# duanyiqun/DiffusionDepth

Hardware: AMD Instinct MI355X
Metric: depth-maps/sec (20-step DDIM, KITTI 352x1216 f16r, B=4 maps per GPU per step; depth RMSE vs the reference's CPU path <= 1e-3 on this workload AND at KITTI's depth range 0-80 m: see cpu_baseline.rmse_gate) (higher is better)
Workload: dtype f16 (f16 MFMA operands, fp32 accumulation; refined mode: f16-pair weights in conv1 / conv4 / conv3(cond), block-scaled int16 hand-over of y3 and conv3(cond)); 1 GPU; kitti 352x1216 image -> latent 16x176x608, cond 256x176x608, Res head denoiser (mmbev_res50 config), T=20, encoder+loop+decoder, inputs resident in HBM; global_batch=4, parallelism=dp1 (independent images, no collective), ranks_seen=1, streams=2, graph=True, variant=res

## Files before the change

### diffusiondepth_amd/csrc/dd_api.cpp

```cpp
#include "dd_api_internal.h"
#include <cstdlib>

namespace ddapi {
thread_local std::string g_create_error;
}


extern "C" {

const char* dd_version(void) { return "ddepth 0.1 gfx950 (hip, mfma bf16/f16/f32 implicit-GEMM conv3x3+GN+ReLU, hipGraph DDIM loop)"; }

const char* dd_last_error(dd_handle_t h) { return h ? h->err.c_str() : g_create_error.c_str(); }

int dd_create(dd_handle_t* out, int device, int variant) {
  if (!out) { g_create_error = "dd_create: out is NULL"; return DD_ERR_INVALID_ARG; }
  *out = nullptr;
  if (variant != DD_VARIANT_RES && variant != DD_VARIANT_SWIN) { g_create_error = "dd_create: unknown variant"; return DD_ERR_INVALID_ARG; }
  int n = 0;
  hipError_t e = hipGetDeviceCount(&n);
  if (e != hipSuccess || n <= 0) {
    g_create_error = std::string("dd_create: no HIP device available (") + (e != hipSuccess ? hipGetErrorString(e) : "count = 0") +
                     "); this library has no CPU fallback";
    return DD_ERR_HIP;
  }
// ... 90 lines not shown
      DD_HIP(hipDeviceSynchronize());
      h->plans.clear(); h->last_once_plan = nullptr;
      h->cond_bufs.clear(); h->fpn_cond.reset(); h->fpn_cond_key[3] = -1; h->fpn_out.reset(); h->fpn_work.reset();
    }
    h->bf16_pure = value != 0;
  }
  else if (k == "naive_wgrad") h->naive_wgrad = value != 0;
  else if (k == "lane_probe") h->lane_probe = value != 0;
  else if (k == "x3_grad_fp32") h->x3_grad_fp32 = value != 0;
  else if (k == "keep_trajectory") h->keep_traj = value != 0;
  else if (k == "use_trajectory") h->use_traj = value;
  else if (k == "adjoint_tiled") h->adjoint_tiled = value != 0;
  else if (k == "streams") h->n_streams = value < 1 ? 1 : (int)value;
  else if (k == "keep_activations_mb") h->keep_act_mb = value < 0 ? 0 : value;
  else if (k == "big_tiles") {
    if (value < -1 || value > 1) return h->fail(DD_ERR_INVALID_ARG, "dd_set_option: big_tiles must be -1 (automatic), 0 or 1");
    if (h->big_tiles != (int)value) { DD_HIP(hipDeviceSynchronize()); h->plans.clear(); h->last_once_plan = nullptr; }
    h->big_tiles = (int)value;
  }
  else if (k == "thin_slots") {
    if (value < 1 || value > 4096) return h->fail(DD_ERR_INVALID_ARG, "dd_set_option: thin_slots must be in [1, 4096]");
    if (h->thin_slots != (int)value) { DD_HIP(hipDeviceSynchronize()); h->plans.clear(); h->last_once_plan = nullptr; }
    h->thin_slots = (int)value;
  }
  else if (k == "one_buffer") {
    if (value < 0 || value > 2) return h->fail(DD_ERR_INVALID_ARG, "dd_set_option: one_buffer must be 0, 1 or 2");
    if (h->one_buffer != (int)value) { DD_HIP(hipDeviceSynchronize()); h->plans.clear(); h->last_once_plan = nullptr; }
    h->one_buffer = (int)value;
  }
  else if (k == "cond_direct") {
    if (value < 0 || value > 1) return h->fail(DD_ERR_INVALID_ARG, "dd_set_option: cond_direct must be 0 or 1");
    h->cond_direct = (int)value;
  }
  else if (k == "cond_split") {
    if (value < 0 || value > 1) return h->fail(DD_ERR_INVALID_ARG, "dd_set_option: cond_split must be 0 or 1");
    h->cond_split = (int)value;
  }
  else if (k == "thin_stream") {
    if (value < 0 || value > 1) return h->fail(DD_ERR_INVALID_ARG, "dd_set_option: thin_stream must be 0 or 1");
    if (h->thin_stream != (int)value) {
      DD_HIP(hipDeviceSynchronize());
      h->plans.clear(); h->last_once_plan = nullptr;
    }
    h->thin_stream = (int)value;
  }
  else if (k == "f16r_wide" || k == "f16r_p4" || k == "f16r_c1") {
    if (value < 0 || value > 1) return h->fail(DD_ERR_INVALID_ARG, "dd_set_option: " + k + " must be 0 or 1");
    int& opt = k == "f16r_wide" ? h->f16r_wide : k == "f16r_c1" ? h->f16r_c1 : h->f16r_p4;
    if (opt != (int)value) { DD_HIP(hipDeviceSynchronize()); h->plans.clear(); h->last_once_plan = nullptr; }
    opt = (int)value;
  }
  else if (k == "phase_prof_buffer") h->prof_buf = reinterpret_cast<unsigned long long*>((uintptr_t)value);
  else if (k == "phase_prof_layer") h->prof_layer = (int)value;
  else if (k == "layer_timing") {
    drain_layer_events(h);
    h->layer_timing = value != 0;
    for (int i = 0; i < dd_handle_s::N_LAYER_SLOTS; ++i) { h->layer_ms[i] = 0; h->layer_cnt[i] = 0; }
  } else return h->fail(DD_ERR_INVALID_ARG, "dd_set_option: unknown key '" + k + "'");
  return DD_OK;
}

int dd_get_counter(dd_handle_t h, const char* key, int64_t* value) {
  if (!h || !key || !value) return DD_ERR_INVALID_ARG;
  const std::string k(key);
  if (k == "graph_launches") *value = h->n_graph_launches;
  else if (k == "graph_default") *value = h->graph_off_by_env ? 0 : 1;
  else if (k == "eager_loops") *value = h->n_eager_loops;
  else if (k == "graph_capture_failures") *value = h->n_capture_failures;
  else if (k == "plans") *value = (int64_t)h->plans.size();
  else if (k == "neck_launches") *value = h->n_neck_launches;
  else if (k == "trajectory_ticket") *value = h->traj_serial;
  else if (k == "lane_calls") *value = h->n_lane_calls;
  else if (k == "lane_probe_retries") *value = h->n_lane_probe_retries;
  else if (k == "lane_overlap") *value = h->lane_overlap_seen;
  else if (k == "cond_split_ok") *value = (h->fpn_committed && h->fpn_split_ok ? 1 : 0) | (h->neck_committed && h->neck_split_ok ? 2 : 0);
  else if (k == "resident_slots") *value = h->resident_slots;
  else if (k == "trajectory_reuses") *value = h->n_traj_reuse;
  else if (k == "thin_stream_launches") *value = h->thin_stream_launches;
  else if (k.compare(0, 13, "kid_launches:") == 0) {
    int id = 0;
    const size_t n = k.size() - 13;
    bool ok = n >= 1 && n <= 3 && !(n > 1 && k[13] == '0');
    for (size_t i = 13; ok && i < k.size(); ++i) { ok = k[i] >= '0' && k[i] <= '9'; id = id * 10 + (k[i] - '0'); }
    if (!ok || !kid_listed(id)) return h->fail(DD_ERR_INVALID_ARG, "dd_get_counter: '" + k + "' does not name a kernel id (dd_kernel_ids.h)");
    *value = h->kid_launches[id];
  }
  else return h->fail(DD_ERR_INVALID_ARG, "dd_get_counter: unknown key '" + k + "'");
  return DD_OK;
}

int dd_get_layer_ms(dd_handle_t h, int layer, double* total_ms, int64_t* launches) {
  if (!h || layer < 1 || layer > dd_handle_s::N_LAYER_SLOTS || !total_ms || !launches) return DD_ERR_INVALID_ARG;
  drain_layer_events(h);
  *total_ms = h->layer_ms[layer - 1];
  *launches = h->layer_cnt[layer - 1];
  return DD_OK;
}

int dd_last_loop_ms(dd_handle_t h, float* ms) {
  if (!h || !ms) return DD_ERR_INVALID_ARG;
  *ms = 0.f;
  if (!h->ev_valid) return DD_OK;
  DD_HIP(hipEventSynchronize(h->ev1));
  DD_HIP(hipEventElapsedTime(ms, h->ev0, h->ev1));
  return DD_OK;
// ... 425 lines not shown
  }
  h->last_once_plan = pl;
  pl->traj_ticket = (h->keep_traj && precision != DD_PREC_NAIVE_FP32) ? ++h->traj_serial : 0;
  pl->traj_weights = h->weights_serial;
  if (h->debug_sync) DD_HIP(hipStreamSynchronize(s));
  return DD_OK;
}

int dd_add_noise(dd_handle_t h, const float* x0, const float* noise, const int64_t* t, float* out, int B, int C,
                 int lat_h, int lat_w, void* stream) {
  if (!h) return DD_ERR_INVALID_ARG;
  if (h->n_train <= 0) return h->fail(DD_ERR_STATE, "schedule not set (dd_set_schedule)");
  if (!x0 || !noise || !t || !out || B <= 0 || C <= 0 || lat_h <= 0 || lat_w <= 0)
    return h->fail(DD_ERR_INVALID_ARG, "dd_add_noise: null pointer or non-positive size");
  DD_HIP(hipSetDevice(h->device));
  DD_HIP(launch_add_noise(x0, noise, reinterpret_cast<const long long*>(t), h->d_acp.as<float>(), h->n_train, out, B,
                          (long long)C * lat_h * lat_w, reinterpret_cast<hipStream_t>(stream)));
  return DD_OK;
}

static int ensure_codec_tmp(dd_handle_t h, size_t bytes) {
  if (h->codec_tmp.bytes >= bytes) return DD_OK;
  DD_HIP(hipDeviceSynchronize());
  DD_HIP(h->codec_tmp.alloc(bytes));
  return DD_OK;
}

int dd_encode(dd_handle_t h, const float* depth, float* latent, int B, int H, int W, void* stream) {
  if (!h) return DD_ERR_INVALID_ARG;
  if (!h->codec_committed) return h->fail(DD_ERR_STATE, "depth_transform.* weights not committed");
  if (!depth || !latent || B <= 0 || H <= 0 || W <= 0) return h->fail(DD_ERR_INVALID_ARG, "dd_encode: null pointer or non-positive size");
  DD_HIP(hipSetDevice(h->device));
  const int lh = (H - 1) / 2 + 1, lw = (W - 1) / 2 + 1;
  int rc = ensure_codec_tmp(h, (size_t)B * lh * lw * LATENT_C * 4);
  if (rc) return rc;
  DD_HIP(launch_encode(h->codec, depth, h->codec_tmp.as<float>(), latent, B, H, W, reinterpret_cast<hipStream_t>(stream)));
  return DD_OK;
}

int dd_decode(dd_handle_t h, const float* latent, float* depth, int B, int lat_h, int lat_w, void* stream) {
  if (!h) return DD_ERR_INVALID_ARG;
  if (!h->codec_committed) return h->fail(DD_ERR_STATE, "depth_transform.* weights not committed");
  if (!latent || !depth || B <= 0 || lat_h <= 0 || lat_w <= 0) return h->fail(DD_ERR_INVALID_ARG, "dd_decode: null pointer or non-positive size");
  DD_HIP(hipSetDevice(h->device));
  int rc = ensure_codec_tmp(h, (size_t)B * (2 * lat_h) * (2 * lat_w) * LATENT_C * 4);
  if (rc) return rc;
  DD_HIP(launch_decode(h->codec, latent, h->codec_tmp.as<float>(), depth, B, lat_h, lat_w, reinterpret_cast<hipStream_t>(stream)));
  return DD_OK;
}

int dd_debug_fetch(dd_handle_t h, const char* name, float* out, int64_t numel, void* stream) {
  if (!h || !name || !out) return DD_ERR_INVALID_ARG;
  Plan* pl = h->last_once_plan;
  if (!pl) return h->fail(DD_ERR_STATE, "dd_debug_fetch: no dd_denoise_once call to inspect");
  const std::string n(name);
  const void* src = nullptr; int C = 0; int ek = store_kind(pl->ek);
  if (n == "y1") { src = pl->y1.p; C = HID_C; }
  else if (n == "y2") { src = pl->y2.p; C = COND_C; }
  else if (n == "y3") {
    src = pl->y3.p; C = HID_C;
    if (pl->ek == EK_F16R && pl->wide) return h->fail(DD_ERR_UNSUPPORTED, "dd_debug_fetch: y3 travels as scaled int16 in this plan (option f16r_wide = 1)");
  }
  else if (n == "y4") { src = pl->y4.p; C = LATENT_C; ek = EK_F32; }
  else return h->fail(DD_ERR_INVALID_ARG, "dd_debug_fetch: unknown tensor '" + n + "'");
  if (numel != (int64_t)pl->key.B * C * pl->key.h * pl->key.w) return h->fail(DD_ERR_INVALID_ARG, "dd_debug_fetch: numel mismatch");
  DD_HIP(launch_nhwc_to_nchw_f32(src, ek, out, pl->key.B, C, pl->key.h, pl->key.w, pl->key.prec != DD_PREC_NAIVE_FP32,
// ... 42 lines not shown
```

### diffusiondepth_amd/csrc/dd_api_internal.h

```cpp
#pragma once
#include "../../include/ddepth.h"
#include "dd_kernels.h"
#include "dd_kernel_ids.h"

#include <cmath>
#include <cstdio>
#include <cstring>
#include <map>
#include <memory>
#include <set>
#include <string>
#include <tuple>
#include <vector>

using namespace dd;

namespace ddapi {

extern thread_local std::string g_create_error;

struct DevBuf {
  void* p = nullptr;
  size_t bytes = 0;
  DevBuf() = default;
// ... 72 lines not shown
  int lane = 0;
  int lanes = 1;
  bool operator<(const PlanKey& o) const {
    return std::tie(B, h, w, ch, cw, T, prec, hoist, keep, lane, lanes) < std::tie(o.B, o.h, o.w, o.ch, o.cw, o.T, o.prec, o.hoist, o.keep, o.lane, o.lanes);
  }
};

struct Plan {
  PlanKey key{};
  int ek = EK_F32;
  DevBuf x[2];
  std::shared_ptr<DevBuf> cond;
  const void* cond_alias = nullptr;
  const void* graph_cond = nullptr;
  void* cond_ptr() const { return cond_alias ? const_cast<void*>(cond_alias) : (cond ? cond->p : nullptr); }
  DevBuf y1, y2, y3, y4;
  DevBuf a1, f, a3, eps;
  DevBuf sa, sf;
  DevBuf bX, bA1, bF, bA3;
  DevBuf bSa, bSf;
  DevBuf xstash;
  int64_t traj_ticket = 0;
  int64_t traj_weights = -1;
  bool traj_consumed = false;
  DevBuf gA, gY;
  DevBuf dgb;
  DevBuf bcorr;
  DevBuf ttab, tt_scratch;
  int64_t ttab_weights = -1;
  DevBuf ccond;
  DevBuf ccond_raw;
  DevBuf ccond_scale;
  DevBuf y3_scale;
  bool wide = false, c1 = false, p4 = false;
  DevBuf stats;
  DevBuf c1c2;
  DevBuf tsteps;
  std::vector<long long> tsteps_host;
  size_t stats_bytes = 0;
  hipGraphExec_t exec = nullptr;
  bool capture_failed = false;
  uint64_t last_use = 0;
  ~Plan() { if (exec) (void)hipGraphExecDestroy(exec); }
  int slots = 1;
  size_t kept_bytes = 0;
  void* slot(const DevBuf& b, int step) const { return static_cast<char*>(b.p) + (slots > 1 ? (size_t)step * (b.bytes / slots) : 0); }
  double* stat_ptr(int step, int layer) const {
    return stats.as<double>() + ((size_t)(step * 4 + layer) * key.B) * STAT_SLOTS * STAT_STRIDE;
  }
};

struct FpnWork {
  int B = 0, ek = -1, pyr = 0, hs[FPN_LEVELS] = {0}, ws[FPN_LEVELS] = {0};
  DevBuf fin[FPN_LEVELS];
  DevBuf lat[FPN_LEVELS];
  DevBuf up[FPN_LEVELS - 1];
  DevBuf pooled[FPN_LEVELS - 1];
  bool neck = false;
  DevBuf nk_cat[FPN_LEVELS];
  DevBuf nk_out[FPN_LEVELS];
};


struct NeckConv { int layer; std::string name; int cout, cin, ks, level, kind, C, Ck; };
constexpr int NECK_C_MPVIT[4] = {128, 216, 288, 288};
inline int neck_c(int pyr, int level) { return pyr == PYR_MPVIT ? NECK_C_MPVIT[level] : (192 << level); }
// ... 28 lines not shown
  ConvLayer L[4];
  ConvLayer LA, LB;
  DevBuf emb;
  DevBuf etab;
  DevBuf w5_oihw, w5pack[NUM_WIMG], pairp, kside;
  int64_t w5_weights = -1;
  int swin_w5 = 1;
  DevBuf zero_bias;
  int hoist_cond = -1;
  bool bf16_pure = false;
  DevBuf codec_buf;
  CodecWeights codec{};
  DevBuf codec_tmp;
  std::vector<float> acp;
  DevBuf d_acp;
  int n_train = 0;
  bool use_graph = true, timing = false, debug_sync = false, layer_timing = false;
  bool graph_off_by_env = false;
  int graph_fence = 0;
  bool train_graphs = false;
  int check_finite = 0;
  DevBuf chk_buf; std::vector<std::string> chk_labels;
  int ablate = 0;
  unsigned long long* prof_buf = nullptr;
  int prof_layer = 0;
  bool keep_traj = false;
  int64_t keep_act_mb = 65536;
  int n_streams = 1;
  int thin_slots = 512;
  int big_tiles = -1;
  int one_buffer = 1;
  int thin_stream = 1;
  int f16r_wide = 1;
  int f16r_c1 = 1;
  int f16r_p4 = 0;
  bool split_ok = true;
  DevBuf wmax;
  int resident_slots = 512;
  hipStream_t lane_stream[MAX_LANES] = {nullptr, nullptr, nullptr, nullptr};
  std::vector<hipEvent_t> probe_events;
  std::vector<hipStream_t> burnt_streams;
  int lane_probe = 1;
  int64_t n_lane_probe_retries = 0, lane_overlap_seen = -1;
  hipEvent_t lane_fork = nullptr, lane_done[MAX_LANES] = {nullptr, nullptr, nullptr, nullptr};
  int64_t n_lane_calls = 0;
  int active_lanes = 1;
  bool adjoint_tiled = true;
  int64_t traj_serial = 0, use_traj = 0, weights_serial = 0, n_traj_reuse = 0;
  int naive_wgrad = 0;
  int x3_grad_fp32 = 0;
  std::map<PlanKey, std::unique_ptr<Plan>> plans;
  DevBuf wgrad_ws[MAX_LANES];
  std::map<std::string, std::unique_ptr<DevBuf>> grads[MAX_LANES];
  std::map<std::tuple<int, int, int, int, int>, std::pair<std::shared_ptr<DevBuf>, uint64_t>> cond_bufs;
  bool neck_committed = false;
  DevBuf neck_w[NECK_CONVS][NUM_WIMG], neck_b[NECK_CONVS];
  int64_t n_neck_launches = 0;
  bool fpn_committed = false;
  int fpn_pyramid = PYR_DEFAULT;
  DevBuf fpn_lat_w[FPN_LEVELS][NUM_WIMG], fpn_lat_b[FPN_LEVELS];
  DevBuf fpn_up_w[FPN_LEVELS - 1][NUM_WIMG], fpn_up_b[FPN_LEVELS - 1];
  std::unique_ptr<FpnWork> fpn_work;
  std::shared_ptr<DevBuf> fpn_out;
  bool fpn_split_ok = false, neck_split_ok = false;
  int cond_direct = 1;
  int cond_split = 1;
  std::shared_ptr<DevBuf> fpn_cond;
  int fpn_cond_key[4] = {0, 0, 0, -1};
  uint64_t tick = 0;
  Plan* last_once_plan = nullptr;
  hipEvent_t ev0 = nullptr, ev1 = nullptr;
  bool ev_valid = false;
  hipStream_t cap_stream = nullptr;
  int64_t n_graph_launches = 0, n_eager_loops = 0, n_capture_failures = 0;
  static constexpr int N_LAYER_SLOTS = KID_LAST;
  double layer_ms[N_LAYER_SLOTS] = {0};
  int64_t layer_cnt[N_LAYER_SLOTS] = {0};
  std::vector<std::tuple<int, hipEvent_t, hipEvent_t>> pending_ev;
// ... 74 lines not shown
```

### diffusiondepth_amd/csrc/dd_api_plans.cpp

```cpp
#include "dd_api_internal.h"

namespace ddapi {

int check_common(dd_handle_t h, int B, int lh, int lw, int ch, int cw, bool need_schedule) {
  if (!h) return DD_ERR_INVALID_ARG;
  if (!h->committed) return h->fail(DD_ERR_STATE, "model.* weights not committed (call dd_set_weight for every key, then dd_commit_weights)");
  if (need_schedule && h->n_train <= 0) return h->fail(DD_ERR_STATE, "schedule not set (dd_set_schedule)");
  if (B <= 0 || lh <= 0 || lw <= 0) return h->fail(DD_ERR_INVALID_ARG, "B, lat_h, lat_w must be positive");
  if (h->variant == DD_VARIANT_RES && (ch != lh || cw != lw))
    return h->fail(DD_ERR_INVALID_ARG, "DD_VARIANT_RES needs cond_h,cond_w == lat_h,lat_w (reference ...res.py:340 adds them elementwise)");
  if (h->variant == DD_VARIANT_SWIN && (ch <= 0 || cw <= 0)) return h->fail(DD_ERR_INVALID_ARG, "cond_h, cond_w must be positive");
  if ((long long)B * lh * lw * COND_C >= (1LL << 31) * 4) return h->fail(DD_ERR_INVALID_ARG, "tensor too large");
  return DD_OK;
}

int lane_count(dd_handle_t h, int B, int precision) {
  int S = h->n_streams;
  if (S > B) S = B;
  if (S > dd_handle_s::MAX_LANES) S = dd_handle_s::MAX_LANES;
  if (precision == DD_PREC_NAIVE_FP32 || h->layer_timing || h->debug_sync || h->prof_buf || h->check_finite) S = 1;
  return S < 1 ? 1 : S;
}

int check_split(dd_handle_t h, int precision, const char* who) {
// ... 105 lines not shown
    if (victim == h->plans.end()) break;
    if (h->last_once_plan == victim->second.get()) h->last_once_plan = nullptr;
    DD_HIP(hipDeviceSynchronize());
    h->plans.erase(victim);
  }
  std::unique_ptr<Plan> pl(new Plan());
  pl->key = key;
  const bool naive = key.prec == DD_PREC_NAIVE_FP32;
  pl->ek = naive ? EK_F32 : ek_of_precision(key.prec, h->bf16_pure);
  if (pl->ek == EK_F16R && !key.hoist)
    return h->fail(DD_ERR_UNSUPPORTED, "DD_PREC_F16R runs the hoisted forward-only plans: for the Swin / MPViT denoiser those exist with option swin_w5 = 1 "
                                       "(dd_denoise / dd_denoise_trace / dd_denoise_once); training plans: DD_PREC_F16");
  const size_t px = (size_t)key.B * key.h * key.w;
  const size_t es = ek_size(pl->ek);
  DD_HIP(pl->x[0].alloc(px * LATENT_C * 4));
  DD_HIP(pl->x[1].alloc(px * LATENT_C * 4));
  if (key.keep) DD_HIP(pl->xstash.alloc((size_t)(key.T > 0 ? key.T : 1) * px * LATENT_C * 4));
  const bool swin = h->variant == DD_VARIANT_SWIN;
  if (!(pl->ek == EK_F16R && !swin && key.hoist)) { int rc = get_cond_buf(h, key.B, key.h, key.w, key.prec, &pl->cond, key.lane); if (rc) return rc; }
  pl->slots = (key.keep == 2 && key.T > 0) ? key.T : 1;
  const size_t ns = (size_t)pl->slots;
  if (swin) {
    const size_t es_s = pl->ek == EK_F16R ? 4 : es;
    DD_HIP(pl->sa.alloc(ns * px * COND_C * es_s)); DD_HIP(pl->sf.alloc(ns * px * COND_C * es_s));
  }
  if (key.hoist)
  {
    PackGeom g3;
    DD_TRY(pack_geom(h, conv3h_kid(h, key), pl->ek, &g3));
    const int th = g3.th;
    DD_HIP(pl->ccond.alloc((size_t)key.B * ((key.h + th - 1) / th) * ((key.w + 31) / 32) * th * 32 * HID_C * 4));
    if (pl->ek == EK_F16R) {
      pl->wide = h->f16r_wide != 0; pl->c1 = h->f16r_c1 != 0; pl->p4 = h->f16r_p4 != 0;
      DD_HIP(pl->ccond_raw.alloc((size_t)key.B * ((key.h + 7) / 8) * ((key.w + 31) / 32) * 8 * 32 * HID_C * 4));
      if (pl->wide) DD_HIP(pl->ccond_scale.alloc((size_t)key.B * ((key.h + th - 1) / th) * ((key.w + 31) / 32) * 4 * 2 * (th / 4) * 4));
    }
  }
  if (key.hoist && swin) {
    const int T1 = key.T > 0 ? key.T : key.B;
    const int RH = key.h < SWIN_TT_AX ? key.h : SWIN_TT_AX, RW = key.w < SWIN_TT_AX ? key.w : SWIN_TT_AX;
    DD_HIP(pl->ttab.alloc((size_t)T1 * SWIN_TT_ROWS * HID_C * 4));
    DD_HIP(pl->tt_scratch.alloc((size_t)T1 * RH * RW * (2 * COND_C + HID_C) * 4));
    if (h->swin_w5) {
      DD_HIP(pl->bcorr.alloc((size_t)key.B * swin_ring_stride(key.h, key.w) * HID_C * 4));
      DD_HIP(hipMemsetAsync(pl->bcorr.p, 0, pl->bcorr.bytes, nullptr));
      DD_HIP(hipStreamSynchronize(nullptr));
    }
  }
  DD_HIP(pl->y1.alloc(ns * px * HID_C * es));
  DD_HIP(pl->y2.alloc(ns * px * COND_C * es));
  DD_HIP(pl->y3.alloc(ns * px * HID_C * es));
  if (pl->ek == EK_F16R && h->f16r_wide) DD_HIP(pl->y3_scale.alloc(ns * px * 4));
  DD_HIP(pl->y4.alloc(ns * px * LATENT_C * 4));
  if (key.keep == 2) pl->kept_bytes = pl->y1.bytes + pl->y2.bytes + pl->y3.bytes + pl->y3_scale.bytes + pl->y4.bytes + pl->sa.bytes + pl->sf.bytes;
  if (naive) {
    DD_HIP(pl->a1.alloc(px * HID_C * 4));
    DD_HIP(pl->f.alloc(px * COND_C * 4));
    DD_HIP(pl->a3.alloc(px * HID_C * 4));
    DD_HIP(pl->eps.alloc(px * LATENT_C * 4));
  }
  const int T = key.T > 0 ? key.T : 1;
  pl->stats_bytes = (size_t)(T + 1) * 4 * key.B * STAT_SLOTS * STAT_STRIDE * sizeof(double);
  DD_HIP(pl->stats.alloc(pl->stats_bytes));
  std::vector<float> c1c2((size_t)T * 2, 0.f);
  std::vector<long long> ts((size_t)T, 0);
  if (key.T > 0) {
    const int ratio = h->n_train / key.T;
// ... 112 lines not shown

int enqueue_naive_eps(dd_handle_t h, Plan* pl, int step, const float* x_in, const long long* tvec, int t_base,
                      int t_bstride, hipStream_t s) {
  const PlanKey& k = pl->key;
  const int B = k.B, hh = k.h, ww = k.w;
  auto L = h->L;
  DD_HIP(launch_naive_conv3x3(x_in, L[0].w_oihw.as<float>(), L[0].bias.as<float>(), pl->y1.as<float>(), B, hh, ww, LATENT_C, HID_C, s));
  DD_HIP(launch_naive_gn_stats(pl->y1.as<float>(), pl->stat_ptr(step, 0), B, hh, ww, HID_C, s));
  DD_HIP(launch_naive_gn_apply(pl->y1.as<float>(), pl->stat_ptr(step, 0), L[0].gamma.as<float>(), L[0].beta.as<float>(),
                               nullptr, nullptr, nullptr, 0, 0, pl->a1.as<float>(), B, hh, ww, HID_C, s));
  DD_HIP(launch_naive_conv3x3(pl->a1.as<float>(), L[1].w_oihw.as<float>(), L[1].bias.as<float>(), pl->y2.as<float>(), B, hh, ww, HID_C, COND_C, s));
  DD_HIP(launch_naive_gn_stats(pl->y2.as<float>(), pl->stat_ptr(step, 1), B, hh, ww, COND_C, s));
  DD_HIP(launch_naive_gn_apply(pl->y2.as<float>(), pl->stat_ptr(step, 1), L[1].gamma.as<float>(), L[1].beta.as<float>(),
                               static_cast<const float*>(pl->cond_ptr()), h->emb.as<float>(), tvec, t_base, t_bstride, pl->f.as<float>(), B, hh, ww, COND_C, s));
  DD_HIP(launch_naive_conv3x3(pl->f.as<float>(), L[2].w_oihw.as<float>(), L[2].bias.as<float>(), pl->y3.as<float>(), B, hh, ww, COND_C, HID_C, s));
  DD_HIP(launch_naive_gn_stats(pl->y3.as<float>(), pl->stat_ptr(step, 2), B, hh, ww, HID_C, s));
  DD_HIP(launch_naive_gn_apply(pl->y3.as<float>(), pl->stat_ptr(step, 2), L[2].gamma.as<float>(), L[2].beta.as<float>(),
                               nullptr, nullptr, nullptr, 0, 0, pl->a3.as<float>(), B, hh, ww, HID_C, s));
  DD_HIP(launch_naive_conv3x3(pl->a3.as<float>(), L[3].w_oihw.as<float>(), L[3].bias.as<float>(), pl->y4.as<float>(), B, hh, ww, HID_C, LATENT_C, s));
  DD_HIP(launch_naive_gn_stats(pl->y4.as<float>(), pl->stat_ptr(step, 3), B, hh, ww, LATENT_C, s));
  DD_HIP(launch_naive_gn_apply(pl->y4.as<float>(), pl->stat_ptr(step, 3), L[3].gamma.as<float>(), L[3].beta.as<float>(),
                               nullptr, nullptr, nullptr, 0, 0, pl->eps.as<float>(), B, hh, ww, LATENT_C, s));
  if (h->debug_sync) DD_HIP(hipStreamSynchronize(s));
  return DD_OK;
}

int enqueue_cond_conv(dd_handle_t h, Plan* pl, hipStream_t s, const float* nchw) {
  const PlanKey& k = pl->key;
  ConvParams p{};
  p.B = k.B; p.h = k.h; p.w = k.w;
  if (pl->ek == EK_F16R) {
    p.in = nchw ? static_cast<const void*>(nchw) : pl->cond_ptr(); p.wpack = h->L[2].wpack2[WIMG_SPLIT].p; p.bias = h->zero_bias.as<float>();
    p.out = pl->ccond_raw.p;
    DD_TRY(launch_conv(h, nchw ? CONV3C_NCHW : KID_CONV3C, EK_F16S, p, s));
    DD_HIP(launch_cadd_reformat(pl->ccond_raw.as<float>(), pl->ccond.p, pl->ccond_scale.as<float>(), k.B, k.h, k.w, plan_big_tiles(h, k) ? 1 : 0, pl->wide ? 2 : 1, s));
    return DD_OK;
  }
  p.in = pl->cond_ptr(); p.wpack = h->L[2].wpack2[wimg_slot(thin_kind(pl->ek))].p; p.bias = h->zero_bias.as<float>(); p.out = pl->ccond.p;
  return launch_conv(h, conv3c_kid(h, k), pl->ek, p, s);
}


int ensure_swin_w5(dd_handle_t h, hipStream_t s) {
  if (h->w5_weights == h->weights_serial) return DD_OK;
  if (!h->LB.w_oihw.p || !h->L[2].w_oihw.p) return h->fail(DD_ERR_STATE, "hoisted Swin form: the fp32 weights of convB / pred.0 are not on the device");
  if (!h->w5_oihw.p) {
    DD_HIP(h->w5_oihw.alloc((size_t)HID_C * COND_C * 25 * 4)); DD_HIP(h->pairp.alloc((size_t)81 * COND_C * HID_C * 4)); DD_HIP(h->kside.alloc(SWIN_KSIDE_BYTES));
  }
  DD_HIP(launch_swin_compose(h->LB.w_oihw.as<float>(), h->L[2].w_oihw.as<float>(), h->w5_oihw.as<float>(), h->pairp.as<float>(), h->kside.p, s));
  for (int wi = 0; wi < NUM_WIMG; ++wi) {
    if (wi == WIMG_STACK) continue;
    const int ekk = wimg_kind(wi);
    PackGeom g5;
    int rc = pack_geom(h, SWIN_PRED5_H, ekk, &g5); if (rc) return rc;
    rc = ensure_bytes(h, h->w5pack[wi], pack_weights_bytes(g5, ekk)); if (rc) return rc;
    DD_HIP(launch_pack_weights(h->w5_oihw.as<float>(), h->w5pack[wi].p, g5, ekk, true, false, s));
  }
  h->w5_weights = h->weights_serial;
  return DD_OK;
}

int enqueue_swin_hoist(dd_handle_t h, Plan* pl, hipStream_t s) {
  const PlanKey& k = pl->key;
  if (k.T > 0 && pl->ttab_weights != h->weights_serial) {
    if (!h->LA.w_oihw.p || !h->LB.w_oihw.p || !h->L[2].w_oihw.p) return h->fail(DD_ERR_STATE, "hoisted Swin form: the fp32 weights of the fuse convolutions are not on the device");
    DD_HIP(launch_swin_ttab(h->LA.w_oihw.as<float>(), h->LB.w_oihw.as<float>(), h->L[2].w_oihw.as<float>(), h->emb.as<float>(),
                            pl->tsteps.as<long long>(), k.T, k.h, k.w, pl->tt_scratch.as<float>(), pl->ttab.as<float>(), s));
    pl->ttab_weights = h->weights_serial;
  }
  if (pl->bcorr.p) { int rc = ensure_swin_w5(h, s); if (rc) return rc; }
  ConvParams p{};
  p.B = k.B; p.h = k.h; p.w = k.w;
  if (pl->ek == EK_F16R) {
    p.in = pl->cond_ptr(); p.wpack = h->LA.wpack2[WIMG_SPLIT].p; p.bias = h->LA.bias.as<float>(); p.out = pl->sa.p;
    DD_TRY(launch_conv(h, KID_SWIN_CONVB, EK_F16S, p, s));
    p.in = pl->sa.p; p.wpack = h->LB.wpack2[WIMG_SPLIT].p; p.bias = h->LB.bias.as<float>(); p.out = pl->sf.p;
    DD_TRY(launch_conv(h, KID_SWIN_CONVB, EK_F16S, p, s));
    p.in = pl->sf.p; p.wpack = h->L[2].wpack2[WIMG_SPLIT].p; p.bias = h->zero_bias.as<float>(); p.out = pl->ccond_raw.p;
    DD_TRY(launch_conv(h, KID_CONV3C, EK_F16S, p, s));
    DD_HIP(launch_cadd_reformat(pl->ccond_raw.as<float>(), pl->ccond.p, pl->ccond_scale.as<float>(), k.B, k.h, k.w, plan_big_tiles(h, k) ? 1 : 0, pl->wide ? 2 : 1, s));
    return DD_OK;
  }
  const int tk = thin_kind(pl->ek);
  p.in = pl->cond_ptr(); p.wpack = h->LA.wpack2[wimg_slot(tk)].p; p.bias = h->LA.bias.as<float>(); p.out = pl->sa.p;
  DD_TRY(launch_conv(h, KID_SWIN_CONVB, tk, p, s));
  p.in = pl->sa.p; p.wpack = h->LB.wpack2[wimg_slot(tk)].p; p.bias = h->LB.bias.as<float>(); p.out = pl->sf.p;
  DD_TRY(launch_conv(h, KID_SWIN_CONVB, tk, p, s));
  p.in = pl->sf.p; p.wpack = h->L[2].wpack2[wimg_slot(tk)].p; p.bias = h->zero_bias.as<float>(); p.out = pl->ccond.p;
  return launch_conv(h, conv3c_kid(h, k), pl->ek, p, s);
}

int stage_condition(dd_handle_t h, Plan* pl, const float* cond, int B, int lat_h, int lat_w, int cond_h, int cond_w,
                    int precision, hipStream_t s, int img0, int whole_B) {
  if (whole_B <= 0) whole_B = B;
  pl->cond_alias = nullptr;
  const bool direct = cond && h->cond_direct && h->variant != DD_VARIANT_SWIN && pl->ek == EK_F16R && pl->key.hoist;
  if (direct) return enqueue_cond_conv(h, pl, s, cond);
  if (!pl->cond) { int rc = get_cond_buf(h, pl->key.B, pl->key.h, pl->key.w, pl->key.prec, &pl->cond, pl->key.lane); if (rc) return rc; }
  if (cond) {
    if (h->variant == DD_VARIANT_SWIN) DD_HIP(launch_upsample_to_blocked(cond, pl->cond->p, cond_kind(pl->ek), B, COND_C, cond_h, cond_w, lat_h, lat_w, s));
    else DD_HIP(launch_nchw_to_nhwc(cond, pl->cond->p, cond_kind(pl->ek), B, COND_C, cond_h, cond_w, precision != DD_PREC_NAIVE_FP32, s));
    if (h->fpn_cond == pl->cond) { h->fpn_cond.reset(); h->fpn_cond_key[3] = -1; }
  } else if (h->variant == DD_VARIANT_SWIN) {
    const int* k = h->fpn_cond_key;
    if (!h->fpn_cond || h->fpn_cond != h->fpn_out || k[0] != whole_B || k[1] != cond_h || k[2] != cond_w || k[3] != precision)
      return h->fail(DD_ERR_STATE, "cond == NULL needs a preceding dd_condition with the same batch, condition size and precision");
    const char* src = static_cast<const char*>(h->fpn_out->p) + (size_t)img0 * COND_C * cond_h * cond_w * ek_size(cond_kind(pl->ek));
    DD_HIP(launch_upsample_blocked(src, pl->cond->p, cond_kind(pl->ek), B, COND_C, cond_h, cond_w, lat_h, lat_w, s));
  } else {
    const int* k = h->fpn_cond_key;
    const bool whole = img0 == 0 && B == whole_B;
    if (!h->fpn_cond || (whole && h->fpn_cond != pl->cond) || k[0] != whole_B || k[1] != lat_h || k[2] != lat_w || k[3] != precision)
      return h->fail(DD_ERR_STATE, "cond == NULL needs a preceding dd_condition with the same batch, latent size and precision");
// ... 43 lines not shown
```

### diffusiondepth_amd/csrc/dd_elem.h

```cpp
#pragma once
#include "dd_kernels.h"
#ifndef DD_NO_PK_F32
#define DD_NO_PK_F32 1
#endif

namespace dd {

constexpr int ACT_CB = 32;
__host__ __device__ inline size_t act_offset(int C, int h, int w, int b, int c, int y, int x) {
  if (C < ACT_CB) return (((size_t)b * h + y) * w + x) * C + c;
  return ((((size_t)b * (C / ACT_CB) + c / ACT_CB) * h + y) * w + x) * ACT_CB + (c % ACT_CB);
}

typedef __attribute__((ext_vector_type(8))) __bf16 bf16x8_t;
typedef __attribute__((ext_vector_type(8))) _Float16 f16x8_t;
typedef __attribute__((ext_vector_type(16))) float f32x16_t;

template <int EK> struct ElemSize { static constexpr int V = (EK == EK_F32) ? 4 : 2; };

__device__ __forceinline__ float bf16_to_f32(uint32_t u16) { return __builtin_bit_cast(float, u16 << 16); }
__device__ __forceinline__ uint32_t f32_to_bf16(float f) {
  uint32_t u = __builtin_bit_cast(uint32_t, f);
  u += 0x7FFFu + ((u >> 16) & 1u);
  return u >> 16;
}
__device__ __forceinline__ float f16_to_f32(uint32_t u16) {
  return (float)__builtin_bit_cast(_Float16, (uint16_t)u16);
}
__device__ __forceinline__ uint32_t f32_to_f16(float f) {
  return (uint32_t)__builtin_bit_cast(uint16_t, (_Float16)f);
}

typedef __attribute__((ext_vector_type(2))) float f32x2_t;
typedef __attribute__((ext_vector_type(2))) __bf16 bf16x2_t;
typedef __attribute__((ext_vector_type(2))) _Float16 f16x2_t;
template <int EK> __device__ __forceinline__ uint32_t pack2(float lo, float hi) {
// ... 8 lines not shown
    const uint32_t w[4] = {v.x, v.y, v.z, v.w};
    if constexpr (EK == EK_F32) {
#pragma unroll
      for (int i = 0; i < 4; ++i) f[i] = __builtin_bit_cast(float, w[i]);
    } else if constexpr (EK == EK_BF16) {
#pragma unroll
      for (int i = 0; i < 4; ++i) { f[2 * i] = bf16_to_f32(w[i] & 0xFFFFu); f[2 * i + 1] = bf16_to_f32(w[i] >> 16); }
    } else {
#pragma unroll
      for (int i = 0; i < 4; ++i) { f[2 * i] = f16_to_f32(w[i] & 0xFFFFu); f[2 * i + 1] = f16_to_f32(w[i] >> 16); }
    }
  }
  static __device__ __forceinline__ uint4 pack(const float (&f)[NE]) {
    uint32_t w[4];
    if constexpr (EK == EK_F32) {
#pragma unroll
      for (int i = 0; i < 4; ++i) w[i] = __builtin_bit_cast(uint32_t, f[i]);
    } else {
#pragma unroll
      for (int i = 0; i < 4; ++i) w[i] = pack2<EK>(f[2 * i], f[2 * i + 1]);
    }
    return make_uint4(w[0], w[1], w[2], w[3]);
  }
};

typedef __attribute__((ext_vector_type(2))) short i16x2_t;
template <int INK, int EK>
__device__ __forceinline__ uint4 affine_relu_pack(const uint4& raw, const float (&ta)[8], const float (&tb)[8]) {
  static_assert(EK != EK_F32 && INK != EK_F32, "2-byte element kinds only");
  const uint32_t w[4] = {raw.x, raw.y, raw.z, raw.w};
  uint32_t o[4];
#pragma unroll
  for (int i = 0; i < 4; ++i) {
    f32x2_t y;
    if constexpr (INK == EK_BF16) { y.x = __builtin_bit_cast(float, w[i] << 16); y.y = __builtin_bit_cast(float, w[i] & 0xFFFF0000u); }
    else { y.x = f16_to_f32(w[i] & 0xFFFFu); y.y = f16_to_f32(w[i] >> 16); }
#if DD_NO_PK_F32
    f32x2_t u;
    u.x = __builtin_fmaf(ta[2 * i], y.x, tb[2 * i]);
    u.y = __builtin_fmaf(ta[2 * i + 1], y.y, tb[2 * i + 1]);
#else
    const f32x2_t a = {ta[2 * i], ta[2 * i + 1]}, b = {tb[2 * i], tb[2 * i + 1]};
    const f32x2_t u = __builtin_elementwise_fma(a, y, b);
#endif
    const i16x2_t pk = __builtin_bit_cast(i16x2_t, pack2<EK>(u.x, u.y));
    const i16x2_t zero = {0, 0};
    o[i] = __builtin_bit_cast(uint32_t, __builtin_elementwise_max(pk, zero));
  }
  return make_uint4(o[0], o[1], o[2], o[3]);
}

template <int EK>
__device__ __forceinline__ void mma_step(f32x16_t& acc, const uint4& wf, const uint4& pf) {
  if constexpr (EK == EK_BF16) {
    acc = __builtin_amdgcn_mfma_f32_32x32x16_bf16(__builtin_bit_cast(bf16x8_t, wf), __builtin_bit_cast(bf16x8_t, pf), acc, 0, 0, 0);
  } else if constexpr (EK == EK_F16) {
    acc = __builtin_amdgcn_mfma_f32_32x32x16_f16(__builtin_bit_cast(f16x8_t, wf), __builtin_bit_cast(f16x8_t, pf), acc, 0, 0, 0);
  } else {
    acc = __builtin_amdgcn_mfma_f32_32x32x2f32(__builtin_bit_cast(float, wf.x), __builtin_bit_cast(float, pf.x), acc, 0, 0, 0);
    acc = __builtin_amdgcn_mfma_f32_32x32x2f32(__builtin_bit_cast(float, wf.y), __builtin_bit_cast(float, pf.y), acc, 0, 0, 0);
    acc = __builtin_amdgcn_mfma_f32_32x32x2f32(__builtin_bit_cast(float, wf.z), __builtin_bit_cast(float, pf.z), acc, 0, 0, 0);
    acc = __builtin_amdgcn_mfma_f32_32x32x2f32(__builtin_bit_cast(float, wf.w), __builtin_bit_cast(float, pf.w), acc, 0, 0, 0);
  }
}

}
// ... 1 lines not shown
```

### diffusiondepth_amd/csrc/dd_igemm2.hip

```cpp
#include "dd_igemm2_cfg.h"
#include "dd_gcn.h"

namespace dd {

#if DD_PHASE_PROF && !defined(DD_HOST_EMULATION)
#define DD_PROF_MARK(i) do { if (p.prof != nullptr && threadIdx.x == 0) p.prof[(size_t)blockIdx.x * 8 + (i)] = (unsigned long long)wall_clock64(); } while (0)
#define DD_PROF_HWID() do { if (p.prof != nullptr && threadIdx.x == 0) {                                                     \
    unsigned hw_, xcc_; asm volatile("s_getreg_b32 %0, hwreg(HW_REG_HW_ID)" : "=s"(hw_)); asm volatile("s_getreg_b32 %0, hwreg(HW_REG_XCC_ID)" : "=s"(xcc_));   \
    p.prof[(size_t)blockIdx.x * 8 + 6] = hw_; p.prof[(size_t)blockIdx.x * 8 + 7] = xcc_; } } while (0)
#define DD_PROF_CLK() ((unsigned long long)__builtin_amdgcn_s_memtime())
#define DD_PROF_LOOP_DECL unsigned long long pl_acc_[4] = {0, 0, 0, 0}, pl_t_ = 0
#define DD_PROF_LOOP_START() do { if (p.prof != nullptr) pl_t_ = DD_PROF_CLK(); } while (0)
#define DD_PROF_LOOP_ADD(k) do { if (p.prof != nullptr) { const unsigned long long n_ = DD_PROF_CLK(); pl_acc_[k] += n_ - pl_t_; pl_t_ = n_; } } while (0)
#define DD_PROF_LOOP_STORE() do { if (p.prof != nullptr && lane == 0) { for (int k_ = 0; k_ < 4; ++k_)                          \
    p.prof[(size_t)gridDim.x * 8 + ((size_t)blockIdx.x * C::WAVES + wave) * 4 + k_] = pl_acc_[k_]; } } while (0)
#else
#define DD_PROF_MARK(i) ((void)0)
#define DD_PROF_HWID() ((void)0)
#define DD_PROF_LOOP_DECL
#define DD_PROF_LOOP_START() ((void)0)
#define DD_PROF_LOOP_ADD(k) ((void)0)
#define DD_PROF_LOOP_STORE() ((void)0)
#endif

// ... 630 lines not shown
          float v[4];
          value_of(n, q, v);
          if (pvalid) {
            const float s = (v[0] + v[1]) + (v[2] + v[3]);
            const float sq = fmaf(v[0], v[0], fmaf(v[1], v[1], fmaf(v[2], v[2], v[3] * v[3])));
            const int lg = 2 * n + (q >> 1);
            ls[lg] += s; lq[lg] += sq;
          }
          pmax = fmaxf(pmax, fmaxf(fmaxf(fabsf(v[0]), fabsf(v[1])), fmaxf(fabsf(v[2]), fabsf(v[3]))));
#pragma unroll
          for (int i = 0; i < 4; ++i) acc[n][m][q * 4 + i] = v[i];
        }
      pmax = fmaxf(pmax, __shfl_xor(pmax, 32, 64));
      const float inv = pmax > 0.f ? 1.f / pmax : 0.f;
      if (pvalid && g == 0) p.out_scale[(size_t)e_b * h * w + (size_t)gy * w + gx] = pmax * (1.f / Q15_ONE);
#pragma unroll
      for (int n = 0; n < C::WN; ++n) {
        uint2 pk[4];
#pragma unroll
        for (int q = 0; q < 4; ++q) {
          pk[q].x = DD_CVT_PKNORM_I16(acc[n][m][q * 4 + 0] * inv, acc[n][m][q * 4 + 1] * inv);
          pk[q].y = DD_CVT_PKNORM_I16(acc[n][m][q * 4 + 2] * inv, acc[n][m][q * 4 + 3] * inv);
        }
#pragma unroll
        for (int k = 0; k < 2; ++k) {
          const auto rx = __builtin_amdgcn_permlane32_swap(pk[2 * k].x, pk[2 * k + 1].x, false, false);
          const auto ry = __builtin_amdgcn_permlane32_swap(pk[2 * k].y, pk[2 * k + 1].y, false, false);
          const int co = n0 + n * 32 + 16 * k + 8 * g;
          if (pvalid) *reinterpret_cast<uint4*>(out_b + act_offset(C::COUT, h, w, 0, co, gy, gx) * 2) = make_uint4(rx[0], ry[0], rx[1], ry[1]);
        }
      }
      continue;
    }
#pragma unroll
    for (int n = 0; n < C::WN; ++n) {
      uint2 pk[4];
#pragma unroll
      for (int q = 0; q < 4; ++q) {
        if (C::COUT < 32 && q >= 2) continue;
        const int co = n0 + n * 32 + 8 * q + 4 * g;
        float v[4];
        value_of(n, q, v);
        if (C::STATS && pvalid) {
          const float s = (v[0] + v[1]) + (v[2] + v[3]);
          const float sq = fmaf(v[0], v[0], fmaf(v[1], v[1], fmaf(v[2], v[2], v[3] * v[3])));
          const int lg = (C::COUT == COND_C) ? (n >> 1) : (C::COUT == HID_C) ? (2 * n + (q >> 1)) : q;
          ls[lg] += s; lq[lg] += sq;
        }
        if constexpr (C::LAYER == KID_CONV3C) {
          const size_t fi = ((((size_t)e_tile * C::WAVES + wave) * C::WN + n) * C::WM + m) * 256 + q * 64 + lane;
          if constexpr (C::CADD16) reinterpret_cast<uint2*>(p.out)[fi] = make_uint2(pack2<EK_F16>(v[0], v[1]), pack2<EK_F16>(v[2], v[3]));
          else reinterpret_cast<float4*>(p.out)[fi] = make_float4(v[0], v[1], v[2], v[3]);
        } else if constexpr (C::OUT_ESZ == 4) {
          if (pvalid && (C::COUT_PAD == C::COUT || co < C::COUT)) {
            if constexpr (C::SCATTER) {
              const int par = co >> 8, cc = co & (COND_C - 1);
              *reinterpret_cast<float4*>(reinterpret_cast<char*>(p.out) + ((size_t)e_b * 4 * h * w * COND_C +
                  act_offset(COND_C, 2 * h, 2 * w, 0, cc, 2 * gy + (par >> 1), 2 * gx + (par & 1))) * 4) = make_float4(v[0], v[1], v[2], v[3]);
            } else {
              *reinterpret_cast<float4*>(out_b + act_offset(C::COUT, h, w, 0, co, gy, gx) * 4) = make_float4(v[0], v[1], v[2], v[3]);
            }
          }
        } else {
          pk[q].x = pack2<C::OUT_K>(v[0], v[1]);
          pk[q].y = pack2<C::OUT_K>(v[2], v[3]);
        }
// ... 119 lines not shown
```

### diffusiondepth_amd/csrc/dd_misc.hip

```cpp
#include "dd_elem.h"
#include "dd_gcn.h"

namespace dd {
__device__ __forceinline__ float relu_keep_nan(float v) { return (v < 0.f) ? 0.f : v; }


__device__ __forceinline__ uint32_t cvt_bf16(float f) {
  uint32_t u = __builtin_bit_cast(uint32_t, f);
  u += 0x7FFFu + ((u >> 16) & 1u);
  return u >> 16;
}
__device__ __forceinline__ uint32_t cvt_f16(float f) { return (uint32_t)__builtin_bit_cast(uint16_t, (_Float16)f); }
__device__ __forceinline__ float ld_elem(const void* base, size_t idx, int ek) {
  if (ek == EK_F32) return reinterpret_cast<const float*>(base)[idx];
  const uint32_t u = reinterpret_cast<const uint16_t*>(base)[idx];
  return ek == EK_BF16 ? __builtin_bit_cast(float, u << 16) : (float)__builtin_bit_cast(_Float16, (uint16_t)u);
}

template <int EK>
__global__ void __launch_bounds__(256) nchw_to_nhwc_kernel(const float* __restrict__ src, void* __restrict__ dst,
                                                           int C, int Cd, long long HW, int blocked) {
  __shared__ float tile[64][65];
  const int b = blockIdx.z;
  const long long p0 = (long long)blockIdx.x * 64;
// ... 724 lines not shown
  };
  fetch(0, cur, cur_in);
#pragma unroll 1
  for (int tap = 0; tap < 9; ++tap) {
    fetch(tap < 8 ? tap + 1 : 8, nx, nx_in);
    float in[LATENT_C];
#pragma unroll
    for (int q = 0; q < 4; ++q) {
      in[4 * q] = cur_in ? cur[q].x : 0.f; in[4 * q + 1] = cur_in ? cur[q].y : 0.f; in[4 * q + 2] = cur_in ? cur[q].z : 0.f; in[4 * q + 3] = cur_in ? cur[q].w : 0.f;
    }
    const float* wt = w1t + (size_t)tap * LATENT_C * LATENT_C;
#pragma unroll
    for (int q = 0; q < LATENT_C / 4; ++q) {
#pragma unroll
      for (int j = 0; j < 4; ++j) {
        const int ci = 4 * q + j;
        const f32x2_t* row = reinterpret_cast<const f32x2_t*>(wt + ci * LATENT_C);
        const f32x2_t a = (f32x2_t){in[ci], in[ci]};
#pragma unroll
        for (int co = 0; co < LATENT_C / 2; ++co) acc[co] = __builtin_elementwise_fma(row[co], a, acc[co]);
      }
      DD_SCHED_FENCE();
    }
#pragma unroll
    for (int q = 0; q < 4; ++q) cur[q] = nx[q];
    cur_in = nx_in;
  }
  if (ok) {
#pragma unroll
    for (int c = 0; c < LATENT_C; ++c) latent[((size_t)b * LATENT_C + c) * HW + p] = tanhf(acc[c >> 1][c & 1]);
  }
}

hipError_t launch_encode(const CodecWeights& cw, const float* depth, float* tmp_nhwc, float* latent_nchw,
                         int B, int H, int W, hipStream_t s) {
  const int h = (H - 1) / 2 + 1, w = (W - 1) / 2 + 1;
  dim3 grid((unsigned)(((long long)h * w + 255) / 256), (unsigned)B);
  hipLaunchKernelGGL(enc0_kernel, grid, dim3(256), 0, s, depth, cw.enc_w0, cw.enc_b0, tmp_nhwc, H, W, h, w);
  hipLaunchKernelGGL(enc1_kernel, grid, dim3(256), 0, s, tmp_nhwc, cw.enc_w1t, cw.enc_b1, latent_nchw, h, w);
  return hipGetLastError();
}

__global__ void __launch_bounds__(256) dec0_kernel(const float* __restrict__ latent, const float* __restrict__ w0,
                                                   const float* __restrict__ b0, float* __restrict__ tmp, int h, int w) {
  const int b = blockIdx.y;
  const int H = 2 * h, W = 2 * w;
  const long long HW = (long long)h * w;
  const long long p = (long long)blockIdx.x * blockDim.x + threadIdx.x;
  if (p >= (long long)H * W) return;
  const int oy = (int)(p / W), ox = (int)(p - (long long)oy * W);
  float acc[LATENT_C];
#pragma unroll
  for (int c = 0; c < LATENT_C; ++c) acc[c] = b0[c];
  const float* lat = latent + (size_t)b * LATENT_C * HW;
#pragma unroll
  for (int a = 0; a < 2; ++a) {
    const int ky = ((oy + 1) & 1) + 2 * a;
    const int iy = (oy + 1 - ky) >> 1;
    if (iy < 0 || iy >= h) continue;
#pragma unroll
    for (int c2 = 0; c2 < 2; ++c2) {
      const int kx = ((ox + 1) & 1) + 2 * c2;
      const int ix = (ox + 1 - kx) >> 1;
      if (ix < 0 || ix >= w) continue;
      for (int ci = 0; ci < LATENT_C; ++ci) {
        const float v = lat[(size_t)ci * HW + (size_t)iy * w + ix];
        const float* wr = w0 + ((size_t)ci * LATENT_C) * 16 + ky * 4 + kx;
#pragma unroll
        for (int co = 0; co < LATENT_C; ++co) acc[co] = fmaf(wr[co * 16], v, acc[co]);
// ... 295 lines not shown
```

Baseline: 549.3 maps/s.

## Fuse encoder convs, fold cond conv3 int16 quantization into epilogue, add f16 mix path

Adds a fused encoder kernel that computes the stride-2 first conv into a shared-memory halo tile and applies the second 3x3 conv from there, removing the NHWC intermediate buffer and one launch. It also quantizes the conv3(cond) output to block-scaled int16 directly in the GEMM epilogue, which skips the separate ccond_raw buffer and the reformat kernel. A DD_MIX16 compile flag adds an f16 packed affine+ReLU path, off by default. The fused encoder recomputes halo pixels, and the epilogue's per-block max reduction adds shuffles and register pressure to the conv kernel.

Result: no change. 553.6 maps/s, median of 6 (+0.8%).

```diff
diff --git a/diffusiondepth_amd/csrc/dd_api.cpp b/diffusiondepth_amd/csrc/dd_api.cpp
--- a/diffusiondepth_amd/csrc/dd_api.cpp
+++ b/diffusiondepth_amd/csrc/dd_api.cpp
@@ -146,6 +146,10 @@
     if (value < 0 || value > 1) return h->fail(DD_ERR_INVALID_ARG, "dd_set_option: cond_direct must be 0 or 1");
     h->cond_direct = (int)value;
   }
+  else if (k == "enc_fused") {
+    if (value < 0 || value > 1) return h->fail(DD_ERR_INVALID_ARG, "dd_set_option: enc_fused must be 0 or 1");
+    h->enc_fused = (int)value;
+  }
   else if (k == "cond_split") {
     if (value < 0 || value > 1) return h->fail(DD_ERR_INVALID_ARG, "dd_set_option: cond_split must be 0 or 1");
     h->cond_split = (int)value;
@@ -158,9 +162,9 @@
     }
     h->thin_stream = (int)value;
   }
-  else if (k == "f16r_wide" || k == "f16r_p4" || k == "f16r_c1") {
+  else if (k == "f16r_wide" || k == "f16r_p4" || k == "f16r_c1" || k == "cadd_fused") {
     if (value < 0 || value > 1) return h->fail(DD_ERR_INVALID_ARG, "dd_set_option: " + k + " must be 0 or 1");
-    int& opt = k == "f16r_wide" ? h->f16r_wide : k == "f16r_c1" ? h->f16r_c1 : h->f16r_p4;
+    int& opt = k == "f16r_wide" ? h->f16r_wide : k == "f16r_c1" ? h->f16r_c1 : k == "cadd_fused" ? h->cadd_fused : h->f16r_p4;
     if (opt != (int)value) { DD_HIP(hipDeviceSynchronize()); h->plans.clear(); h->last_once_plan = nullptr; }
     opt = (int)value;
   }
@@ -185,6 +189,8 @@
   else if (k == "neck_launches") *value = h->n_neck_launches;
   else if (k == "trajectory_ticket") *value = h->traj_serial;
   else if (k == "lane_calls") *value = h->n_lane_calls;
+  else if (k == "cadd_reformat_launches") *value = h->n_cadd_reformat;
+  else if (k == "enc_fused_launches") *value = h->n_enc_fused;
   else if (k == "lane_probe_retries") *value = h->n_lane_probe_retries;
   else if (k == "lane_overlap") *value = h->lane_overlap_seen;
   else if (k == "cond_split_ok") *value = (h->fpn_committed && h->fpn_split_ok ? 1 : 0) | (h->neck_committed && h->neck_split_ok ? 2 : 0);
@@ -676,6 +682,11 @@
   if (!depth || !latent || B <= 0 || H <= 0 || W <= 0) return h->fail(DD_ERR_INVALID_ARG, "dd_encode: null pointer or non-positive size");
   DD_HIP(hipSetDevice(h->device));
   const int lh = (H - 1) / 2 + 1, lw = (W - 1) / 2 + 1;
+  if (h->enc_fused) {
+    DD_HIP(launch_encode(h->codec, depth, nullptr, latent, B, H, W, reinterpret_cast<hipStream_t>(stream)));
+    h->n_enc_fused++;
+    return DD_OK;
+  }
   int rc = ensure_codec_tmp(h, (size_t)B * lh * lw * LATENT_C * 4);
   if (rc) return rc;
   DD_HIP(launch_encode(h->codec, depth, h->codec_tmp.as<float>(), latent, B, H, W, reinterpret_cast<hipStream_t>(stream)));
diff --git a/diffusiondepth_amd/csrc/dd_api_internal.h b/diffusiondepth_amd/csrc/dd_api_internal.h
--- a/diffusiondepth_amd/csrc/dd_api_internal.h
+++ b/diffusiondepth_amd/csrc/dd_api_internal.h
@@ -128,6 +128,7 @@
   DevBuf ccond_raw;
   DevBuf ccond_scale;
   DevBuf y3_scale;
+  bool cadd_fused = false;
   bool wide = false, c1 = false, p4 = false;
   DevBuf stats;
   DevBuf c1c2;
@@ -222,6 +223,8 @@
   int one_buffer = 1;
   int thin_stream = 1;
   int f16r_wide = 1;
+  int enc_fused = 1;
+  int cadd_fused = 1;
   int f16r_c1 = 1;
   int f16r_p4 = 0;
   bool split_ok = true;
@@ -234,6 +237,7 @@
   int64_t n_lane_probe_retries = 0, lane_overlap_seen = -1;
   hipEvent_t lane_fork = nullptr, lane_done[MAX_LANES] = {nullptr, nullptr, nullptr, nullptr};
   int64_t n_lane_calls = 0;
+  int64_t n_cadd_reformat = 0, n_enc_fused = 0;
   int active_lanes = 1;
   bool adjoint_tiled = true;
   int64_t traj_serial = 0, use_traj = 0, weights_serial = 0, n_traj_reuse = 0;
diff --git a/diffusiondepth_amd/csrc/dd_api_plans.cpp b/diffusiondepth_amd/csrc/dd_api_plans.cpp
--- a/diffusiondepth_amd/csrc/dd_api_plans.cpp
+++ b/diffusiondepth_amd/csrc/dd_api_plans.cpp
@@ -161,7 +161,8 @@
     DD_HIP(pl->ccond.alloc((size_t)key.B * ((key.h + th - 1) / th) * ((key.w + 31) / 32) * th * 32 * HID_C * 4));
     if (pl->ek == EK_F16R) {
       pl->wide = h->f16r_wide != 0; pl->c1 = h->f16r_c1 != 0; pl->p4 = h->f16r_p4 != 0;
-      DD_HIP(pl->ccond_raw.alloc((size_t)key.B * ((key.h + 7) / 8) * ((key.w + 31) / 32) * 8 * 32 * HID_C * 4));
+      pl->cadd_fused = pl->wide && h->cadd_fused && th == 8;
+      if (!pl->cadd_fused) DD_HIP(pl->ccond_raw.alloc((size_t)key.B * ((key.h + 7) / 8) * ((key.w + 31) / 32) * 8 * 32 * HID_C * 4));
       if (pl->wide) DD_HIP(pl->ccond_scale.alloc((size_t)key.B * ((key.h + th - 1) / th) * ((key.w + 31) / 32) * 4 * 2 * (th / 4) * 4));
     }
   }
@@ -340,8 +341,11 @@
   if (pl->ek == EK_F16R) {
     p.in = nchw ? static_cast<const void*>(nchw) : pl->cond_ptr(); p.wpack = h->L[2].wpack2[WIMG_SPLIT].p; p.bias = h->zero_bias.as<float>();
     p.out = pl->ccond_raw.p;
+    if (pl->cadd_fused) { p.out = pl->ccond.p; p.out_scale = pl->ccond_scale.as<float>(); }
     DD_TRY(launch_conv(h, nchw ? CONV3C_NCHW : KID_CONV3C, EK_F16S, p, s));
+    if (pl->cadd_fused) return DD_OK;
     DD_HIP(launch_cadd_reformat(pl->ccond_raw.as<float>(), pl->ccond.p, pl->ccond_scale.as<float>(), k.B, k.h, k.w, plan_big_tiles(h, k) ? 1 : 0, pl->wide ? 2 : 1, s));
+    h->n_cadd_reformat++;
     return DD_OK;
   }
   p.in = pl->cond_ptr(); p.wpack = h->L[2].wpack2[wimg_slot(thin_kind(pl->ek))].p; p.bias = h->zero_bias.as<float>(); p.out = pl->ccond.p;
@@ -385,8 +389,11 @@
     p.in = pl->sa.p; p.wpack = h->LB.wpack2[WIMG_SPLIT].p; p.bias = h->LB.bias.as<float>(); p.out = pl->sf.p;
     DD_TRY(launch_conv(h, KID_SWIN_CONVB, EK_F16S, p, s));
     p.in = pl->sf.p; p.wpack = h->L[2].wpack2[WIMG_SPLIT].p; p.bias = h->zero_bias.as<float>(); p.out = pl->ccond_raw.p;
+    if (pl->cadd_fused) { p.out = pl->ccond.p; p.out_scale = pl->ccond_scale.as<float>(); }
     DD_TRY(launch_conv(h, KID_CONV3C, EK_F16S, p, s));
+    if (pl->cadd_fused) return DD_OK;
     DD_HIP(launch_cadd_reformat(pl->ccond_raw.as<float>(), pl->ccond.p, pl->ccond_scale.as<float>(), k.B, k.h, k.w, plan_big_tiles(h, k) ? 1 : 0, pl->wide ? 2 : 1, s));
+    h->n_cadd_reformat++;
     return DD_OK;
   }
   const int tk = thin_kind(pl->ek);
diff --git a/diffusiondepth_amd/csrc/dd_elem.h b/diffusiondepth_amd/csrc/dd_elem.h
--- a/diffusiondepth_amd/csrc/dd_elem.h
+++ b/diffusiondepth_amd/csrc/dd_elem.h
@@ -2,6 +2,9 @@
 #include "dd_kernels.h"
 #ifndef DD_NO_PK_F32
 #define DD_NO_PK_F32 1
+#endif
+#ifndef DD_MIX16
+#define DD_MIX16 0
 #endif
 
 namespace dd {
@@ -76,6 +79,21 @@
   uint32_t o[4];
 #pragma unroll
   for (int i = 0; i < 4; ++i) {
+#if DD_MIX16
+    if constexpr (INK == EK_F16 && EK == EK_F16) {
+      const f16x2_t yh = __builtin_bit_cast(f16x2_t, w[i]);
+      f16x2_t r;
+      r.x = (_Float16)__builtin_fmaf(ta[2 * i], (float)yh.x, tb[2 * i]);
+      r.y = (_Float16)__builtin_fmaf(ta[2 * i + 1], (float)yh.y, tb[2 * i + 1]);
+      uint32_t rw = __builtin_bit_cast(uint32_t, r);
+#ifndef DD_HOST_EMULATION
+      asm("" : "+v"(rw));
+#endif
+      const i16x2_t zero = {0, 0};
+      o[i] = __builtin_bit_cast(uint32_t, __builtin_elementwise_max(__builtin_bit_cast(i16x2_t, rw), zero));
+      continue;
+    }
+#endif
     f32x2_t y;
     if constexpr (INK == EK_BF16) { y.x = __builtin_bit_cast(float, w[i] << 16); y.y = __builtin_bit_cast(float, w[i] & 0xFFFF0000u); }
     else { y.x = f16_to_f32(w[i] & 0xFFFFu); y.y = f16_to_f32(w[i] >> 16); }
diff --git a/diffusiondepth_amd/csrc/dd_igemm2.hip b/diffusiondepth_amd/csrc/dd_igemm2.hip
--- a/diffusiondepth_amd/csrc/dd_igemm2.hip
+++ b/diffusiondepth_amd/csrc/dd_igemm2.hip
@@ -686,6 +686,33 @@
       }
       continue;
     }
+    if constexpr (C::LAYER == KID_CONV3C && C::SPLIT) {
+      if (p.out_scale != nullptr) {
+        auto nmax = [](float a, float b) { return (b > a || b != b) ? b : a; };
+#pragma unroll
+        for (int n = 0; n < C::WN; ++n) {
+          float mx = 0.f;
+#pragma unroll
+          for (int q = 0; q < 4; ++q) {
+            float v[4];
+            value_of(n, q, v);
+            mx = nmax(mx, nmax(nmax(fabsf(v[0]), fabsf(v[1])), nmax(fabsf(v[2]), fabsf(v[3]))));
+#pragma unroll
+            for (int i = 0; i < 4; ++i) acc[n][m][q * 4 + i] = v[i];
+          }
+#pragma unroll
+          for (int off = 32; off >= 1; off >>= 1) mx = nmax(mx, __shfl_xor(mx, off, 64));
+          const float inv = mx > 0.f ? 1.f / mx : 0.f;
+          const size_t blk = (((size_t)e_tile * C::WAVES + wave) * C::WN + n) * C::WM + m;
+          if (lane == 0) p.out_scale[blk] = mx * (1.f / Q15_ONE);
+#pragma unroll
+          for (int q = 0; q < 4; ++q)
+            reinterpret_cast<uint2*>(p.out)[blk * 256 + q * 64 + lane] =
+                make_uint2(DD_CVT_PKNORM_I16(acc[n][m][q * 4 + 0] * inv, acc[n][m][q * 4 + 1] * inv), DD_CVT_PKNORM_I16(acc[n][m][q * 4 + 2] * inv, acc[n][m][q * 4 + 3] * inv));
+        }
+        continue;
+      }
+    }
 #pragma unroll
     for (int n = 0; n < C::WN; ++n) {
       uint2 pk[4];
diff --git a/diffusiondepth_amd/csrc/dd_misc.hip b/diffusiondepth_amd/csrc/dd_misc.hip
--- a/diffusiondepth_amd/csrc/dd_misc.hip
+++ b/diffusiondepth_amd/csrc/dd_misc.hip
@@ -780,9 +780,83 @@
   }
 }
 
+constexpr int ET_H = 8, ET_W = 32;
+constexpr int ER_H = ET_H + 2, ER_W = ET_W + 2, ER_P = ER_W + 1;
+__global__ void __launch_bounds__(256) enc_fused_kernel(const float* __restrict__ depth, const float* __restrict__ w0, const float* __restrict__ b0,
+                                                        const float* __restrict__ w1t, const float* __restrict__ b1, float* __restrict__ latent,
+                                                        int H, int W, int h, int w) {
+  static_assert(ET_H * ET_W == 256, "one latent pixel per thread");
+  __shared__ float s_mid[LATENT_C][ER_H][ER_P];
+  const int b = blockIdx.z;
+  const int Y0 = blockIdx.y * ET_H, X0 = blockIdx.x * ET_W;
+  const int tid = threadIdx.x;
+  const float* d = depth + (size_t)b * H * W;
+  for (int i = tid; i < ER_H * ER_W; i += 256) {
+    const int r = i / ER_W, c = i - r * ER_W;
+    const int oy = Y0 - 1 + r, ox = X0 - 1 + c;
+    if (oy >= 0 && oy < h && ox >= 0 && ox < w) {
+      float in[9];
+#pragma unroll
+      for (int ky = 0; ky < 3; ++ky)
+#pragma unroll
+        for (int kx = 0; kx < 3; ++kx) {
+          const int iy = 2 * oy - 1 + ky, ix = 2 * ox - 1 + kx;
+          in[ky * 3 + kx] = (iy >= 0 && iy < H && ix >= 0 && ix < W) ? d[(size_t)iy * W + ix] : 0.f;
+        }
+#pragma unroll
+      for (int ch = 0; ch < LATENT_C; ++ch) {
+        float a = b0[ch];
+#pragma unroll
+        for (int k = 0; k < 9; ++k) a = fmaf(w0[ch * 9 + k], in[k], a);
+        s_mid[ch][r][c] = a >= 0.f ? a : 0.2f * a;
+      }
+    } else {
+#pragma unroll
+      for (int ch = 0; ch < LATENT_C; ++ch) s_mid[ch][r][c] = 0.f;
+    }
+  }
+  __syncthreads();
+  const int ty = tid >> 5, tx = tid & 31;
+  const int oy = Y0 + ty, ox = X0 + tx;
+  f32x2_t acc[LATENT_C / 2];
+#pragma unroll
+  for (int c = 0; c < LATENT_C / 2; ++c) acc[c] = (f32x2_t){b1[2 * c], b1[2 * c + 1]};
+#pragma unroll 1
+  for (int tap = 0; tap < 9; ++tap) {
+    const int ky = tap / 3, kx = tap - ky * 3;
+    float in[LATENT_C];
+#pragma unroll
+    for (int ci = 0; ci < LATENT_C; ++ci) in[ci] = s_mid[ci][ty + ky][tx + kx];
+    const float* wt = w1t + (size_t)tap * LATENT_C * LATENT_C;
+#pragma unroll
+    for (int q = 0; q < LATENT_C / 4; ++q) {
+#pragma unroll
+      for (int j = 0; j < 4; ++j) {
+        const int ci = 4 * q + j;
+        const f32x2_t* row = reinterpret_cast<const f32x2_t*>(wt + ci * LATENT_C);
+        const f32x2_t a = (f32x2_t){in[ci], in[ci]};
+#pragma unroll
+        for (int co = 0; co < LATENT_C / 2; ++co) acc[co] = __builtin_elementwise_fma(row[co], a, acc[co]);
+      }
+      DD_SCHED_FENCE();
+    }
+  }
+  if (oy < h && ox < w) {
+    const long long HW = (long long)h * w;
+    const long long p = (long long)oy * w + ox;
+#pragma unroll
+    for (int c = 0; c < LATENT_C; ++c) latent[((size_t)b * LATENT_C + c) * HW + p] = tanhf(acc[c >> 1][c & 1]);
+  }
+}
+
 hipError_t launch_encode(const CodecWeights& cw, const float* depth, float* tmp_nhwc, float* latent_nchw,
                          int B, int H, int W, hipStream_t s) {
   const int h = (H - 1) / 2 + 1, w = (W - 1) / 2 + 1;
+  if (tmp_nhwc == nullptr) {
+    dim3 grid((unsigned)((w + ET_W - 1) / ET_W), (unsigned)((h + ET_H - 1) / ET_H), (unsigned)B);
+    hipLaunchKernelGGL(enc_fused_kernel, grid, dim3(256), 0, s, depth, cw.enc_w0, cw.enc_b0, cw.enc_w1t, cw.enc_b1, latent_nchw, H, W, h, w);
+    return hipGetLastError();
+  }
   dim3 grid((unsigned)(((long long)h * w + 255) / 256), (unsigned)B);
   hipLaunchKernelGGL(enc0_kernel, grid, dim3(256), 0, s, depth, cw.enc_w0, cw.enc_b0, tmp_nhwc, H, W, h, w);
   hipLaunchKernelGGL(enc1_kernel, grid, dim3(256), 0, s, tmp_nhwc, cw.enc_w1t, cw.enc_b1, latent_nchw, h, w);
```
